# Healthcare-Robotics/assistive-gym

Measured on NVIDIA H100. Metric: env-steps/sec FeedingJaco-v1 @batch4096, higher is better.
Workload: dtype f32

## Files before the change

assistive_gym_b200/csrc/ag_solver.cuh:

```cuda
#pragma once
#include "ag_device.cuh"

#define RS_HDR 16
#define RS_LB 32
#define RS_UNIT 16
#define RS_MAXREC (RS_HDR + 4 * RS_LB)
enum { RM_BOX = 0, RM_CONE = 1, RM_PAD = 2 };

struct alignas(16) v4 { float x, y, z, w; };
AG_HD v4 ldv4(const float* p) { return *(const v4*)p; }
AG_HD void stv4(float* p, v4 a) { *(v4*)p = a; }
AG_HD float i2f_bits(int v) { float f; memcpy(&f, &v, 4); return f; }
AG_HD int f2i_bits(float f) { int v; memcpy(&v, &f, 4); return v; }

AG_HD int rs_null(const SimDev& S) { return S.NDp + 8 * S.nf; }
AG_HD int rs_nv(const SimDev& S) { return (S.NDp + 8 * S.nf + 8 + 31) & ~31; }
AG_HD int rs_dummy(const SimDev& S) { return 3 * S.ND + S.ngr + 3 * S.maxc; }
AG_HD int rs_nlam(const SimDev& S) { return (3 * S.ND + S.ngr + 3 * S.maxc + 1 + 31) & ~31; }
#define RS_CTA_ENVS 8
AG_HD int rs_env_floats(const SimDev& S) { return rs_nv(S) + rs_nlam(S) + 64 + 1024; }
AG_HD int rs_env_stride(const SimDev& S) { return rs_nv(S) + rs_nlam(S) + 8; }
AG_HD int rs_cta_floats(const SimDev& S) { return 1024 + RS_CTA_ENVS * (1024 + rs_env_stride(S)) + 2 * RS_CTA_ENVS; }

AG_HD int link_ref(const SimDev& S, int e, int link) {
// ... 143 lines not shown
  if (kind < 2) {
    if (!AG_LDG(S.link_haslimit + k)) return false;
    if (kind == 0) { float pen = q - AG_LDG(S.link_lower + k); if (pen > 0.f) return false; R.rhs = (-pen * S.erp / dt - qd) * R.dinv; }
    else { float pen = AG_LDG(S.link_upper + k) - q; if (pen > 0.f) return false; R.rhs = (-pen * S.erp / dt + qd) * R.dinv; R.sgn = -1.f; }
  } else {
    int mode = S.motor_mode[k];
    float maxi = S.motor_maxf[k] * dt;
    if (S.motor_fscale) maxi *= ld1(S.motor_fscale, k, N, e);
    if (mode == 0 || !(maxi > 0.f)) return false;
    float vt = (mode == 1) ? (S.motor_kp[k] * (ld1(S.motor_target, k, N, e) - q) / dt + qd - S.motor_kd[k] * qd)
                           : ld1(S.motor_target, k, N, e);
    R.rhs = (vt - qd) * R.dinv; R.lo = -maxi; R.hi = maxi;
  }
  return true;
}
AG_HD bool con_sides(const SimDev& S, int e, int c, int& refA, int& refB, bool& swapped) {
  const int N = S.N;
  int ka = AG_LDG(S.con_link + 2 * c), kb = AG_LDG(S.con_link + 2 * c + 1);
  int ba = AG_LDG(S.link_body + ka), bb = AG_LDG(S.link_body + kb);
  if (S.body_mode[(size_t)ba * N + e] == 0 || S.body_mode[(size_t)bb * N + e] == 0) return false;
  refA = link_ref(S, e, ka); refB = link_ref(S, e, kb);
  swapped = rs_swap_sides(refA, refB);
  if (swapped) { int t = refA; refA = refB; refB = t; }
  return ((refA | refB) & 3) != 0;
}

AG_HD void contact_refs(const SimDev& S, int e, unsigned key, int& refA, int& refB) {
  unsigned pairk = key >> 2;
  int ca = (int)(pairk / (unsigned)S.nc), cb = (int)(pairk % (unsigned)S.nc);
  refA = link_ref(S, e, AG_LDG(S.col_link + ca)); refB = link_ref(S, e, AG_LDG(S.col_link + cb));
  if (rs_swap_sides(refA, refB)) { int t = refA; refA = refB; refB = t | (1 << 30); }
}

AG_HDN inline void rows_body(int e, const SimDev& S, const KP&) {
  const int N = S.N;
  RsCur c; c.pos = 0; c.rs = S.rs_data + (size_t)e * S.rs_cap; c.capf = S.rs_cap; c.over = false;
  int open_key = -1, open_row = -1, open_off = -1;
  for (int pass = 0; pass < 2; pass++) {
    for (int d = 0; d < S.ND; d++) {
      for (int kind = (pass == 0 ? 0 : 2); kind < (pass == 0 ? 2 : 3); kind++) {
        const int r = kind * S.ND + d;
        DofRow R;
        int info = -1;
        if (dof_row(S, e, kind, d, R)) {
          int a = AG_LDG(S.dl_art + d);
          int key = 0x10000 | a;
          if (open_key == key) {
            info = rs_enc(open_off, 1, 1);
            S.row_off[(size_t)open_row * N + e] |= 2; S.row_pair[(size_t)open_row * N + e] = r;
            open_key = -1;
          } else {
            int nd = AG_LDG(S.art_nd + a);
            int o = rs_alloc(S, c, rs_rec_floats(nd > 8 ? 2 : 1));
            if (o >= 0) { info = rs_enc(o, 0, 0); open_key = key; open_row = r; open_off = o; }
          }
        }
        S.row_off[(size_t)r * N + e] = info;
        S.row_pair[(size_t)r * N + e] = -1;
      }
    }
  }
  open_key = -1;
  for (int cc = 0; cc < S.ncon; cc++) {
    int refA, refB; bool sw;
    bool on = con_sides(S, e, cc, refA, refB, sw);
    RsShape h; h.nv = 0;
    if (on) h = rs_shape(S, refA, refB);
    for (int i = 0; i < 6; i += 2) {
      int r = 3 * S.ND + 6 * cc + i;
      int i0 = -1, i1 = -1;
      if (on && h.nv > 0) {
        int o = rs_alloc(S, c, rs_rec_floats(h.nv));
        if (o >= 0) { i0 = rs_enc(o, 0, 1); i1 = rs_enc(o, 1, 1); }
      }
      S.row_off[(size_t)r * N + e] = i0; S.row_off[(size_t)(r + 1) * N + e] = i1;
      S.row_pair[(size_t)r * N + e] = i0 >= 0 ? r + 1 : -1; S.row_pair[(size_t)(r + 1) * N + e] = -1;
    }
  }
  int cnt = S.c_count[e]; if (cnt > S.maxc) cnt = S.maxc;
  int open_slot = -1;
  for (int s = 0; s < cnt; s++) {
    size_t rb = (size_t)s * 4 * N + e;
    int refA = S.s_ref[rb], refB = S.s_ref[rb + N] & ~(1 << 30);
    RsShape h = rs_shape(S, refA, refB);
    int key = rs_shape_key(h);
    int info = -1;
    if (key >= 0) {
      if (open_key == key && open_slot == s - 1) {
        info = rs_enc(open_off, 1, 1);
        S.s_ref[(size_t)(s - 1) * 4 * N + e + 2 * (size_t)N] |= 2;
        open_key = -1;
      } else {
        int o = rs_alloc(S, c, rs_rec_floats(h.nv));
        if (o >= 0) { info = rs_enc(o, 0, 0); open_key = key; open_slot = s; open_off = o; }
      }
    } else open_key = -1;
    S.s_ref[rb + 2 * (size_t)N] = info;
  }
  for (int s = 0; s < cnt; s++) {
    size_t rb = (size_t)s * 4 * N + e;
    int refA = S.s_ref[rb], refB = S.s_ref[rb + N] & ~(1 << 30);
    RsShape h = rs_shape(S, refA, refB);
    int o = -1;
    if (h.nv > 0 && S.s_ref[rb + 2 * (size_t)N] >= 0) o = rs_alloc(S, c, rs_rec_floats(h.nv));
    S.s_ref[rb + 3 * (size_t)N] = o < 0 ? -1 : o / RS_UNIT;
  }
  if (c.pos % 32 != 0) {
    if (c.pos + RS_UNIT <= c.capf) { rs_pad_header(S, c.rs + c.pos, RM_PAD, RS_UNIT); c.pos += RS_UNIT; } else c.over = true;
  }
  S.rs_nfloats[e] = c.over ? (c.pos / 32) * 32 : c.pos;
  if (c.over) S.overflow[e] = 1;
}

AG_HD void rs_finish_box(const SimDev& S, float* rec, int nv, int row, int li, float num, float lo, float hi) {
  float diag = rs_row_diag(rec, nv, row);
  if (diag > 1e-20f) { float dinv = 1.0f / diag; rs_set_row(S, rec, row, li, num * dinv, dinv, lo, hi); }
  else rs_null_row(rec, nv, row);
}

AG_HDN inline void drow_body(int r, int e, const SimDev& S) {
  const int N = S.N;
  const float dt = S.dt;
  int info = S.row_off[(size_t)r * N + e];
  if (info < 0 || (info & 1)) return;
  float* rec = S.rs_data + (size_t)e * S.rs_cap + (size_t)(info >> 2) * RS_UNIT;
  const int r2 = (info & 2) ? S.row_pair[(size_t)r * N + e] : -1;
  if (r < 3 * S.ND) {
    int d = r % S.ND;
    int a = AG_LDG(S.dl_art + d), d0 = AG_LDG(S.art_dl0 + a), nd = AG_LDG(S.art_nd + a), vo = AG_LDG(S.art_voff + a);
    RsShape h; h.nv = nd > 8 ? 2 : 1; h.sl[0] = vo; h.sl[1] = nd > 8 ? vo + 8 : rs_null(S); h.sl[2] = h.sl[3] = rs_null(S);
    rs_header(S, rec, h, RM_BOX);
    rs_zero_blocks(rec, h.nv);
    int dd[2] = {d, 0}; float sg[2] = {1.f, 1.f};
    for (int row = 0; row < (r2 >= 0 ? 2 : 1); row++) {
      int rr = row == 0 ? r : r2;
      int kind = rr / S.ND; dd[row] = rr % S.ND;
      DofRow R;
      if (!dof_row(S, e, kind, dd[row], R)) continue;
      sg[row] = R.sgn;
      for (int i = 0; i < nd; i++) {
        float* q = rs_entry(rec, 0, i, row);
        q[0] = (i == dd[row] - d0) ? R.sgn : 0.f;
        q[1] = R.sgn * S.Minv[((size_t)(d0 + i) * S.ND + dd[row]) * N + e];
      }
// ... 593 lines not shown
```

assistive_gym_b200/csrc/ag_types.h:

```cpp
#pragma once
#include <stdint.h>
#include <stddef.h>

#define AG_MAXND 16
#define AG_MAX_HULL 64
#define AG_CF 20
#define AG_CFR 10

enum {
  CF_PAX = 0, CF_PAY, CF_PAZ, CF_PBX, CF_PBY, CF_PBZ, CF_NX, CF_NY, CF_NZ, CF_DIST,
  CF_RHS_N, CF_DINV_N, CF_RHS_T1, CF_DINV_T1, CF_RHS_T2, CF_DINV_T2, CF_MU, CF_LAM_N, CF_LAM_T1, CF_LAM_T2
};
enum { BK_STATIC = 0, BK_FREE = 1, BK_ART = 2 };

struct SimDev {
  int N;
  float dt; int iters; float erp, contact_erp, slop, resid_thr, contact_thr, lin_damp, ang_damp, vmax;
  int cone, gyro, maxc;
  int nb, nl, nc, npair, ncon, nf, nart, ND, nparts, nmovcol, nmovlink, nalllink, ngr ;
  const int *body_link0, *body_nlinks, *body_kind, *body_idx;
  const float* body_gravity;
  const int *link_body, *link_parent, *link_jtype, *link_dl, *link_haslimit, *link_col0, *link_ncol;
  const float *link_axis, *link_jpos, *link_jquat, *link_com, *link_iquat, *link_inertia, *link_mass, *link_lower, *link_upper;
  const int *col_link, *col_type, *col_v0, *col_nv, *col_p0, *col_np;
// ... 6 lines not shown
  const int* con_link; const float *con_pivot, *con_quat, *con_maxforce;
  const int* free_body; const float* free_invm;
  const int *art_body, *art_dl0, *art_nd, *art_voff;
  int NDp;
  const int *dl_link, *dl_parent, *dl_type, *dl_art, *dl_part0, *dl_nparts;
  const float *dl_mass, *dl_mc, *dl_J, *dl_damping;
  const float *pt_mass, *pt_com, *pt_I;
  int* motor_mode; float *motor_kp, *motor_kd, *motor_maxf;
  int* hard_limit;
  float *motor_target, *motor_applied;
  float* motor_fscale;
  float *base_pos, *base_quat, *base_lin, *base_ang;
  float *jq, *jqd;
  float* friction;
  int* body_mode;
  float *lpos, *lquat;
  float *cmin, *cmax, *lmin, *lmax;
  int* cand_count; unsigned *cand, *cand_s; int maxcand;
  int* c_count;
  int maxraw;
  unsigned *c_key, *s_key;
  float *c_data, *s_data;
  int *s_ref;
  int* overflow;
  float *fcom, *fIinv;
  float *jax, *jor;
  float* Minv;
  float* dv;
  float* dr_lam;
  float* gr_lam;
  int* row_off;
  int* row_pair;
  float* rs_data; int rs_cap; int* rs_nfloats;
  int* iters_used;
  int* pgs_order;
  int* pgs_cycles;
  int* pgs_trips;
};

struct KP {
  int n;
  int i0, i1, i2, i3;
  float f0, f1;
  const void* p0; void* p1; void* p2; void* p3; void* p4; void* p5;
};
```

assistive_gym_b200/csrc/agphys.cu:

```cuda
#include <stdio.h>
#include <stdlib.h>
#include <string.h>
#include <string>
#include <vector>
#include <algorithm>
#include "../../include/agphys.h"
#include "ag_device.cuh"
#include "ag_solver.cuh"
#include "ag_feeding.cuh"
#include "ag_bathing.cuh"
#include "ag_ik.cuh"
#include "ag_cloth.cuh"
#include "ag_dressing.cuh"
#include "ag_render.cuh"
#include "ag_scratch.cuh"
#include "ag_coop.cuh"
#include "ag_drinking.cuh"

#ifndef AG_CPU_EMU
#include <cuda_runtime.h>
#define AG_GLOBAL __global__
#else
#define AG_GLOBAL
typedef void* cudaStream_t;
#endif

static thread_local std::string g_err;
static int fail(const std::string& m) { g_err = m; return -1; }

#ifndef AG_CPU_EMU
#define AG_KERNEL(name, body)                                                   \
  __global__ void __launch_bounds__(128) name(SimDev S, KP p) {                 \
    int tid = blockIdx.x * blockDim.x + threadIdx.x;                            \
    if (tid < p.n) body(tid, S, p);                                             \
  }
#else
#define AG_KERNEL(name, body) \
  static void name(SimDev S, KP p) { for (int tid = 0; tid < p.n; tid++) body(tid, S, p); }
#endif

#ifndef AG_CPU_EMU
#define AG_KERNEL_B(name, body, minblocks)                                      \
  __global__ void __launch_bounds__(128, minblocks) name(SimDev S, KP p) {      \
    int tid = blockIdx.x * blockDim.x + threadIdx.x;                            \
    if (tid < p.n) body(tid, S, p);                                             \
  }
#else
#define AG_KERNEL_B(name, body, minblocks) AG_KERNEL(name, body)
#endif
AG_KERNEL(k_fk, fk_body)
AG_KERNEL(k_aabb, aabb_body)
AG_KERNEL(k_linkaabb, linkaabb_body)
AG_KERNEL(k_pairs, pairs_body)
AG_KERNEL(k_csort, csort_body)
AG_KERNEL_B(k_narrow, narrow_body, 3)
AG_KERNEL(k_sort, sort_body)
AG_KERNEL(k_dyn, dyn_body)
AG_KERNEL(k_rows, rows_body)
AG_KERNEL(k_crows, crows_body)
#ifndef AG_CPU_EMU
__global__ void __launch_bounds__(32) k_pgs(SimDev S, KP p) {
  extern __shared__ __align__(128) float pgs_smem[];
  pgs_warp(S, pgs_smem, p.i0, blockIdx.x * RS_CTA_ENVS);
}
__global__ void __launch_bounds__(1024) k_order(SimDev S, KP) {
  __shared__ int hist[64];
  if (threadIdx.x < 64) hist[threadIdx.x] = 0;
  __syncthreads();
  for (int e = threadIdx.x; e < S.N; e += blockDim.x) atomicAdd(&hist[pgs_work_bucket(S, e)], 1);
  __syncthreads();
  if (threadIdx.x == 0) { int acc = 0; for (int b = 0; b < 64; b++) { int c = hist[b]; hist[b] = acc; acc += c; } }
  __syncthreads();
  for (int e = threadIdx.x; e < S.N; e += blockDim.x) S.pgs_order[atomicAdd(&hist[pgs_work_bucket(S, e)], 1)] = e;
}
#else
static void k_pgs(SimDev S, KP p) {
  std::vector<float> buf((size_t)rs_env_floats(S) + 8);
  float* base = (float*)(((uintptr_t)buf.data() + 15) & ~(uintptr_t)15);
  static const bool emul = getenv("AG_EMU_PLAIN_PGS") == nullptr;
  for (int tid = 0; tid < p.n; tid++) { if (emul) pgs_env_emul(tid, S, base); else pgs_body_host(tid, S, base); }
}
static void k_order(SimDev S, KP) {
  int hist[64] = {0};
  for (int e = 0; e < S.N; e++) hist[pgs_work_bucket(S, e)]++;
  int acc = 0; for (int b = 0; b < 64; b++) { int c = hist[b]; hist[b] = acc; acc += c; }
  for (int e = 0; e < S.N; e++) S.pgs_order[hist[pgs_work_bucket(S, e)]++] = e;
}
#endif
AG_KERNEL(k_integrate, integrate_body)
AG_KERNEL(k_gather, gather_body)
AG_KERNEL(k_scatter, scatter_body)
// ... 49 lines not shown
  const CoopDev& C = *(const CoopDev*)p.p1;
  float h[2 * AG_MLP_H];
  for (int e = 0; e < p.n; e++) coop_limits_body(e, S, C, C.mlp, h, 1);
}
static void k_coop_classify(SimDev, KP p) {
  float h[2 * AG_MLP_H];
  for (int i = 0; i < p.n; i++) {
    const float* xi = (const float*)p.p0 + (size_t)i * 4;
    float x[4] = {xi[0], xi[1], xi[2], xi[3]};
    ((float*)p.p3)[i] = coop_mlp((const float*)p.p2, x, h, 1);
  }
}
#endif

enum Task { TASK_FEEDING = 0, TASK_SCRATCH = 1, TASK_BATHING = 2, TASK_DRESSING = 3, TASK_DRINKING = 4 };
static const int IO_COOP = 5;
static const int ROBOT_OBS_W[5] = {25, 30, 24, 24, 25}, HUMAN_OBS_W[5] = {23, 34, 28, 28, 0};
static const char* const TASK_INIT[5] = {"ag_feeding_init", "ag_scratch_init", "ag_bathing_init", "ag_dressing_init", "ag_drinking_init"};

struct StepOut { float *obs, *obs_h, *reward, *done, *info; };
struct StepGraph { void* exec; const void* key[6]; uint64_t launches; bool valid; };
struct StepIO {
  int act_w, obs_w, obs_h_w;
  float *action, *obs, *obs_h, *reward, *done, *info;
  float *host_in, *host_out;
  StepGraph graph;
};

struct AgSim {
  SimDev S;
  AgConfig cfg;
  int device;
  cudaStream_t stream;
  uint64_t launches;
  std::vector<void*> allocs;
  std::vector<int> body_link0, body_nlinks, body_kind, link_body;
  int nl, nb;
  float* d_stage; size_t stage_floats;
  std::vector<float> h_stage;
  int* d_mask; int* d_links; int* d_icount;
  FeedDev F; FeedDev* F_dev; bool feeding;
  BathDev B; BathDev* B_dev; bool bathing;
  bool bath_frames;
  ClothDev C; ClothDev* C_dev; bool cloth; int cloth_sub, cloth_npt, cloth_qs;
  DressPost DP; DressPost* DP_dev; bool dressing;
  ScratchDev SD; ScratchDev* SD_dev; bool scratch;
  DrinkDev DK; DrinkDev* DK_dev; bool drinking;
  size_t render_pix; int render_n; int* d_render_ids; unsigned char* d_render_rgba; float* d_render_depth; void* d_render_dev;
  CoopDev CO; CoopDev* CO_dev; bool coop;
  StepIO io[6];
  bool use_graph; int graph_failures;
  bool profiling;
  std::vector<std::string> knames;
  std::vector<int> ev_slot;
  std::vector<void*> ev_begin, ev_end;
};

#ifndef AG_CPU_EMU
#define CK(x) do { cudaError_t err__ = (x); if (err__ != cudaSuccess) { g_err = std::string(#x) + ": " + cudaGetErrorString(err__); return -1; } } while (0)
#define CKP(x) do { cudaError_t err__ = (x); if (err__ != cudaSuccess) { g_err = std::string(#x) + ": " + cudaGetErrorString(err__); return nullptr; } } while (0)
#endif

static void drop_graph(StepIO& io) {
#ifndef AG_CPU_EMU
  if (io.graph.valid) { cudaGraphExecDestroy((cudaGraphExec_t)io.graph.exec); io.graph.valid = false; }
#else
// ... 21 lines not shown
#else
  (void)s; memcpy(d, h, bytes);
#endif
  return 0;
}
static int d2h(AgSim* s, void* h, const void* d, size_t bytes) {
#ifndef AG_CPU_EMU
  CK(cudaMemcpyAsync(h, d, bytes, cudaMemcpyDeviceToHost, s->stream));
  CK(cudaStreamSynchronize(s->stream));
#else
  (void)s; memcpy(h, d, bytes);
#endif
  return 0;
}
static int dev_zero(AgSim* s, void* d, size_t bytes) {
#ifndef AG_CPU_EMU
  CK(cudaMemsetAsync(d, 0, bytes, s->stream));
#else
  (void)s; memset(d, 0, bytes);
#endif
  return 0;
}
template <typename T>
static const T* upload(AgSim* s, const std::vector<T>& v) {
  T* d = (T*)dev_alloc(s, v.size() * sizeof(T));
  if (d && !v.empty()) h2d(s, d, v.data(), v.size() * sizeof(T));
  return d;
}
template <typename T>
static T* dalloc(AgSim* s, size_t n) { return (T*)dev_alloc(s, n * sizeof(T)); }

#define AG_MAX_KNAMES 32
static int prof_slot(AgSim* s, const char* name);
static void prof_mark(AgSim* s, int slot, bool begin);
#ifndef AG_CPU_EMU
#define LAUNCH(sim, kern, nthreads, kp)                                                     \
  do {                                                                                      \
    KP kp__ = (kp); kp__.n = (int)(nthreads);                                               \
    if (kp__.n > 0) {                                                                       \
      int ps__ = (sim)->profiling ? prof_slot((sim), #kern) : -1;                           \
      if (ps__ >= 0) prof_mark((sim), ps__, true);                                          \
      kern<<<(kp__.n + 127) / 128, 128, 0, (sim)->stream>>>((sim)->S, kp__);                \
      if (ps__ >= 0) prof_mark((sim), ps__, false);                                         \
      (sim)->launches++;                                                                    \
    }                                                                                       \
  } while (0)
#else
#define LAUNCH(sim, kern, nthreads, kp) \
  do { KP kp__ = (kp); kp__.n = (int)(nthreads); if (kp__.n > 0) { kern((sim)->S, kp__); (sim)->launches++; } } while (0)
#endif

static int prof_slot(AgSim* s, const char* name) {
  for (size_t i = 0; i < s->knames.size(); i++) if (s->knames[i] == name) return (int)i;
  if (s->knames.size() >= AG_MAX_KNAMES) return -1;
  s->knames.push_back(name);
  return (int)s->knames.size() - 1;
}
static void prof_mark(AgSim* s, int slot, bool begin) {
#ifndef AG_CPU_EMU
  cudaEvent_t ev;
  if (cudaEventCreate(&ev) != cudaSuccess) return;
  cudaEventRecord(ev, s->stream);
  if (begin) { s->ev_slot.push_back(slot); s->ev_begin.push_back((void*)ev); } else s->ev_end.push_back((void*)ev);
#else
  (void)s; (void)slot; (void)begin;
#endif
}

static KP kp0() { KP p; memset(&p, 0, sizeof(p)); return p; }

struct DevGuard {
  int prev;
  explicit DevGuard(int device) : prev(-1) {
#ifndef AG_CPU_EMU
    if (cudaGetDevice(&prev) != cudaSuccess) prev = -1;
    if (prev != device) cudaSetDevice(device); else prev = -1;
#else
    (void)device;
#endif
  }
  ~DevGuard() {
#ifndef AG_CPU_EMU
    if (prev >= 0) cudaSetDevice(prev);
#endif
  }
};

struct HQ { double x, y, z, w; };
static HQ hq_mul(HQ a, HQ b) {
  return HQ{a.w * b.x + a.x * b.w + a.y * b.z - a.z * b.y, a.w * b.y - a.x * b.z + a.y * b.w + a.z * b.x,
            a.w * b.z + a.x * b.y - a.y * b.x + a.z * b.w, a.w * b.w - a.x * b.x - a.y * b.y - a.z * b.z};
}
static void hq_mat(HQ q, double R[9]) {
  double x = q.x, y = q.y, z = q.z, w = q.w;
  R[0] = 1 - 2 * (y * y + z * z); R[1] = 2 * (x * y - z * w); R[2] = 2 * (x * z + y * w);
  R[3] = 2 * (x * y + z * w); R[4] = 1 - 2 * (x * x + z * z); R[5] = 2 * (y * z - x * w);
  R[6] = 2 * (x * z - y * w); R[7] = 2 * (y * z + x * w); R[8] = 1 - 2 * (x * x + y * y);
}

extern "C" {

const char* ag_last_error(void) { return g_err.c_str(); }

void ag_default_config(AgConfig* c) {
  c->dt = 0.02; c->num_substeps = 1; c->num_solver_iters = 50; c->erp = 0.2; c->contact_erp = 0.08;
  c->linear_slop = 1e-5; c->residual_threshold = 1e-7; c->contact_threshold = 0.02;
  c->linear_damping = 0.04; c->angular_damping = 0.04; c->max_coord_velocity = 100; c->hull_margin = 0.001;
  c->cone_friction = 1; c->gyroscopic = 1; c->max_contacts = 128;
  c->warmstart_contact = 0.0; c->warmstart_joint = 0.0;
}

AgSim* ag_create(const AgSceneDesc* d, const AgConfig* cfg, int n_envs, int device) {
  if (!d || !cfg || n_envs <= 0) { g_err = "ag_create: bad arguments"; return nullptr; }
  DevGuard guard__(device);
  AgSim* s = new AgSim();
  memset(&s->S, 0, sizeof(SimDev));
  memset(&s->F, 0, sizeof(FeedDev));
  s->cfg = *cfg; s->device = device; s->launches = 0; s->feeding = false; s->bathing = false; s->cloth = false; s->cloth_sub = 0; s->C_dev = nullptr; s->dressing = false; s->DP_dev = nullptr; s->scratch = false; s->SD_dev = nullptr; s->drinking = false; s->DK_dev = nullptr; s->render_pix = 0; s->render_n = 0; s->d_render_ids = nullptr; s->d_render_rgba = nullptr; s->d_render_depth = nullptr; s->d_render_dev = nullptr; s->use_graph = true; s->graph_failures = 0; s->coop = false; s->CO_dev = nullptr; s->B_dev = nullptr; s->stream = nullptr; s->F_dev = nullptr; s->profiling = false;
  s->d_stage = nullptr; s->stage_floats = 0;
#ifndef AG_CPU_EMU
  { int ndev = 0; if (cudaGetDeviceCount(&ndev) != cudaSuccess || device < 0 || device >= ndev) { g_err = "no such CUDA device (is a CUDA device present? there is no CPU fallback)"; delete s; return nullptr; } }
  if (cudaStreamCreateWithFlags(&s->stream, cudaStreamNonBlocking) != cudaSuccess) { g_err = "cudaStreamCreate failed"; delete s; return nullptr; }
#endif
  SimDev& S = s->S;
  const int N = n_envs;
  S.N = N;
  int sub = cfg->num_substeps > 0 ? cfg->num_substeps : 1;
  S.dt = (float)(cfg->dt / sub); S.iters = cfg->num_solver_iters; S.erp = (float)cfg->erp; S.contact_erp = (float)cfg->contact_erp;
  S.slop = (float)cfg->linear_slop; S.resid_thr = (float)cfg->residual_threshold; S.contact_thr = (float)cfg->contact_threshold;
  S.lin_damp = (float)cfg->linear_damping; S.ang_damp = (float)cfg->angular_damping; S.vmax = (float)cfg->max_coord_velocity;
  S.cone = cfg->cone_friction; S.gyro = cfg->gyroscopic; S.maxc = cfg->max_contacts > 0 ? cfg->max_contacts : 128;
  const int nb = d->n_bodies, nl = d->n_links, nc = d->n_colliders;
  S.nb = nb; S.nl = nl; S.nc = nc; S.npair = d->n_pairs; S.ncon = d->n_constraints;
  s->nb = nb; s->nl = nl;
  s->body_link0.assign(d->body_link0, d->body_link0 + nb);
  s->body_nlinks.assign(d->body_nlinks, d->body_nlinks + nb);
  s->link_body.assign(d->link_body, d->link_body + nl);

  std::vector<double> subtree(nl, 0.0);
  for (int k = nl - 1; k >= 0; k--) { subtree[k] += d->link_mass[k]; if (d->link_parent[k] >= 0) subtree[d->link_parent[k]] += subtree[k]; }
  std::vector<int> live(nl, 0), link_dl(nl, -1), body_kind(nb, BK_STATIC), body_idx(nb, -1);
  std::vector<int> free_body, art_body, art_dl0, art_nd, dl_link, dl_parent, dl_type, dl_art, dl_part0, dl_nparts;
  std::vector<float> dl_mass, dl_mc, dl_J, dl_damping, pt_mass, pt_com, pt_I;
  for (int b = 0; b < nb; b++) {
    int l0 = d->body_link0[b], nlk = d->body_nlinks[b];
    int nlive = 0;
    for (int k = l0 + 1; k < l0 + nlk; k++) {
      int jt = d->link_jtype[k];
      if ((jt == AG_JOINT_REVOLUTE || jt == AG_JOINT_PRISMATIC) && subtree[k] > 0) { live[k] = 1; nlive++; }
    }
    if (d->link_jtype[l0] == AG_JOINT_FREE_BASE && d->link_mass[l0] > 0) {
      if (nlive > 0) { g_err = "floating-base articulated bodies are not supported yet"; ag_destroy(s); return nullptr; }
      body_kind[b] = BK_FREE; body_idx[b] = (int)free_body.size(); free_body.push_back(b);
    } else if (nlive > 0) {
      body_kind[b] = BK_ART; body_idx[b] = (int)art_body.size();
// ... 128 lines not shown
  S.dl_link = upload(s, dl_link); S.dl_parent = upload(s, dl_parent); S.dl_type = upload(s, dl_type); S.dl_art = upload(s, dl_art);
  S.dl_part0 = upload(s, dl_part0); S.dl_nparts = upload(s, dl_nparts);
  S.dl_mass = upload(s, dl_mass); S.dl_mc = upload(s, dl_mc); S.dl_J = upload(s, dl_J); S.dl_damping = upload(s, dl_damping);
  S.pt_mass = upload(s, pt_mass); S.pt_com = upload(s, pt_com); S.pt_I = upload(s, pt_I);
  S.hard_limit = dalloc<int>(s, nl);
  S.motor_mode = dalloc<int>(s, nl); S.motor_kp = dalloc<float>(s, nl); S.motor_kd = dalloc<float>(s, nl); S.motor_maxf = dalloc<float>(s, nl);
  S.motor_target = dalloc<float>(s, (size_t)nl * N); S.motor_applied = dalloc<float>(s, (size_t)nl * N);
  S.base_pos = dalloc<float>(s, (size_t)nb * 3 * N); S.base_quat = dalloc<float>(s, (size_t)nb * 4 * N);
  S.base_lin = dalloc<float>(s, (size_t)nb * 3 * N); S.base_ang = dalloc<float>(s, (size_t)nb * 3 * N);
  S.jq = dalloc<float>(s, (size_t)nl * N); S.jqd = dalloc<float>(s, (size_t)nl * N);
  S.friction = dalloc<float>(s, (size_t)nl * N); S.body_mode = dalloc<int>(s, (size_t)nb * N);
  S.lpos = dalloc<float>(s, (size_t)nl * 3 * N); S.lquat = dalloc<float>(s, (size_t)nl * 4 * N);
  S.cmin = dalloc<float>(s, (size_t)nc * 3 * N); S.cmax = dalloc<float>(s, (size_t)nc * 3 * N);
  S.lmin = dalloc<float>(s, (size_t)nl * 3 * N); S.lmax = dalloc<float>(s, (size_t)nl * 3 * N);
  S.c_count = dalloc<int>(s, N); S.overflow = dalloc<int>(s, N); S.iters_used = dalloc<int>(s, N); S.pgs_cycles = dalloc<int>(s, N); S.pgs_trips = dalloc<int>(s, N);
  S.pgs_order = dalloc<int>(s, N);
  S.maxcand = 4 * S.maxc; S.cand_count = dalloc<int>(s, N); S.cand = dalloc<unsigned>(s, (size_t)S.maxcand * N); S.cand_s = dalloc<unsigned>(s, (size_t)S.maxcand * N);
  if ((size_t)nc * nc >= (1u << 24)) { g_err = "too many colliders (pair id must fit 24 bits)"; ag_destroy(s); return nullptr; }
  S.maxraw = 4 * S.maxc;
  S.c_key = dalloc<unsigned>(s, (size_t)S.maxraw * N); S.s_key = dalloc<unsigned>(s, (size_t)S.maxc * N);
  S.c_data = dalloc<float>(s, (size_t)S.maxraw * AG_CFR * N); S.s_data = dalloc<float>(s, (size_t)S.maxc * AG_CF * N);
  S.s_ref = dalloc<int>(s, (size_t)S.maxc * 4 * N);
  S.fcom = dalloc<float>(s, (size_t)S.nf * 3 * N); S.fIinv = dalloc<float>(s, (size_t)S.nf * 6 * N);
  S.jax = dalloc<float>(s, (size_t)S.ND * 3 * N); S.jor = dalloc<float>(s, (size_t)S.ND * 3 * N);
  S.Minv = dalloc<float>(s, (size_t)S.ND * S.ND * N);
  S.dv = dalloc<float>(s, (size_t)(S.ND + 6 * S.nf) * N);
  S.dr_lam = dalloc<float>(s, (size_t)3 * S.ND * N);
  {
    size_t fl = (size_t)(3 * S.ND / 2 + 2) * rs_rec_floats(2) + (size_t)3 * S.ncon * rs_rec_floats(3) + (size_t)S.maxc * 2 * rs_rec_floats(2);
    fl = fl + fl * 3 / 10 + 1024;
    S.rs_cap = (int)((fl + 1023) / 1024 * 1024);
  }
  if (rs_nv(S) + 8 >= 65536 || rs_nlam(S) >= 65536) { g_err = "solver index space exceeds 16 bits: lower max_contacts"; ag_destroy(s); return nullptr; }
  S.rs_data = dalloc<float>(s, (size_t)S.rs_cap * N); S.rs_nfloats = dalloc<int>(s, N);
  S.gr_lam = dalloc<float>(s, (size_t)S.ngr * N); S.row_off = dalloc<int>(s, (size_t)(3 * S.ND + S.ngr) * N); S.row_pair = dalloc<int>(s, (size_t)(3 * S.ND + S.ngr) * N);
  s->d_mask = dalloc<int>(s, N); s->d_links = dalloc<int>(s, 1024); s->d_icount = dalloc<int>(s, N);
  if (!S.gr_lam || !S.rs_data || !S.rs_nfloats || !S.row_pair || !S.s_data) { g_err = "device allocation failed"; ag_destroy(s); return nullptr; }
#ifndef AG_CPU_EMU
  {
    { const char* gg = getenv("AG_GRAPH"); if (gg && atoi(gg) == 0) s->use_graph = false; }
    size_t smem = (size_t)rs_cta_floats(S) * sizeof(float);
    if (smem > 227 * 1024) { g_err = "PGS shared-memory footprint exceeds 227 KB per CTA: lower max_contacts"; ag_destroy(s); return nullptr; }
    if (cudaFuncSetAttribute(k_pgs, cudaFuncAttributeMaxDynamicSharedMemorySize, (int)smem) != cudaSuccess) { g_err = "cudaFuncSetAttribute(k_pgs) failed"; ag_destroy(s); return nullptr; }
  }
#endif
  {
    std::vector<float> fr((size_t)nl * N);
    for (int k = 0; k < nl; k++) for (int e = 0; e < N; e++) fr[(size_t)k * N + e] = (float)d->link_friction[k];
    h2d(s, S.friction, fr.data(), fr.size() * sizeof(float));
    std::vector<int> md((size_t)nb * N, 1);
    h2d(s, S.body_mode, md.data(), md.size() * sizeof(int));
    std::vector<float> q((size_t)nb * 4 * N, 0.f);
    for (int b = 0; b < nb; b++) for (int e = 0; e < N; e++) q[((size_t)b * 4 + 3) * N + e] = 1.f;
    h2d(s, S.base_quat, q.data(), q.size() * sizeof(float));
  }
  return s;
}

void ag_destroy(AgSim* s) {
  if (!s) return;
  DevGuard guard__(s->device);
#ifndef AG_CPU_EMU
  if (s->stream) cudaStreamSynchronize(s->stream);
  for (void* p : s->allocs) cudaFree(p);
  for (StepIO& io : s->io) {
    cudaFreeHost(io.host_in); cudaFreeHost(io.host_out);
    if (io.graph.valid) cudaGraphExecDestroy((cudaGraphExec_t)io.graph.exec);
  }
  if (s->stream) cudaStreamDestroy(s->stream);
#else
  for (void* p : s->allocs) free(p);
  for (StepIO& io : s->io) { free(io.host_in); free(io.host_out); }
#endif
  delete s;
}

int ag_num_envs(const AgSim* s) {
  DevGuard guard__(s->device); return s->S.N; }
void* ag_stream(AgSim* s) {
  DevGuard guard__(s->device); return (void*)s->stream; }
uint64_t ag_kernel_launches(const AgSim* s) {
  DevGuard guard__(s->device); return s->launches; }

int ag_profile_enable(AgSim* s, int on) {
  DevGuard guard__(s->device);
  s->profiling = on != 0;
  return 0;
}
int ag_profile_get(AgSim* s, int max_names, char* names, int name_stride, float* total_ms, int32_t* counts) {
  DevGuard guard__(s->device);
  int n = (int)s->knames.size();
  if (n > max_names) n = max_names;
  for (int i = 0; i < n; i++) { total_ms[i] = 0.f; counts[i] = 0; snprintf(names + (size_t)i * name_stride, name_stride, "%s", s->knames[i].c_str()); }
#ifndef AG_CPU_EMU
  CK(cudaStreamSynchronize(s->stream));
  size_t m = std::min(s->ev_begin.size(), s->ev_end.size());
  for (size_t i = 0; i < m; i++) {
    float ms = 0.f;
    cudaEventElapsedTime(&ms, (cudaEvent_t)s->ev_begin[i], (cudaEvent_t)s->ev_end[i]);
    int sl = s->ev_slot[i];
    if (sl < n) { total_ms[sl] += ms; counts[sl] += 1; }
// ... 123 lines not shown
  if (h2d(s, s->S.motor_mode, mm.data(), sizeof(int) * s->nl) || h2d(s, s->S.motor_kp, a.data(), sizeof(float) * s->nl) ||
      h2d(s, s->S.motor_kd, b.data(), sizeof(float) * s->nl) || h2d(s, s->S.motor_maxf, c.data(), sizeof(float) * s->nl)) return -1;
  if (target) return scatter_host(s, s->S.motor_target, 1, n, links, target, nullptr);
  return 0;
}
int ag_set_motor_force_scale(AgSim* s, int n, const int32_t* links, const float* scale) {
  DevGuard guard__(s->device);
  if (!s->S.motor_fscale) {
    const size_t cnt = (size_t)s->nl * s->S.N;
    s->S.motor_fscale = dalloc<float>(s, cnt);
    if (!s->S.motor_fscale) return fail("device allocation failed");
    std::vector<float> ones(cnt, 1.0f);
    if (h2d(s, s->S.motor_fscale, ones.data(), cnt * sizeof(float))) return -1;
    drop_all_graphs(s);
  }
  return scatter_host(s, s->S.motor_fscale, 1, n, links, scale, nullptr);
}
int ag_set_motor_targets_dev(AgSim* s, int n, const int32_t* links, const float* target_dev) {
  DevGuard guard__(s->device);
  if (n > 1024) return fail("too many items");
  if (check_items(s, s->S.motor_target, n, links)) return -1;
  if (h2d(s, s->d_links, links, sizeof(int) * n)) return -1;
  KP p = kp0(); p.i0 = 1; p.i1 = n; p.p0 = target_dev; p.p1 = s->S.motor_target; p.p2 = s->d_links; p.p3 = nullptr;
  LAUNCH(s, k_scatter, (size_t)s->S.N * n, p);
  return 0;
}

int ag_set_motor_targets_host(AgSim* s, int n, const int32_t* links, const float* target) {
  DevGuard guard__(s->device);
  return scatter_host(s, s->S.motor_target, 1, n, links, target, nullptr);
}

static void cloth_launch(AgSim* s);
static void substep(AgSim* s) {
  SimDev& S = s->S;
  const int N = S.N;
  KP z = kp0();
  LAUNCH(s, k_fk, (size_t)S.nb * N, z);
  if (s->cloth) {
    KP cs = kp0(); cs.p0 = s->C_dev; cs.i0 = s->cloth_sub;
    LAUNCH(s, k_cloth_snap, (size_t)s->C.ncl * N, cs);
  }
  KP a = kp0(); a.p0 = S.movcol; a.i0 = S.nmovcol;
  LAUNCH(s, k_aabb, (size_t)S.nmovcol * N, a);
  KP l = kp0(); l.p0 = S.movlink; l.i0 = S.nmovlink;
  LAUNCH(s, k_linkaabb, (size_t)S.nmovlink * N, l);
  dev_zero(s, S.c_count, sizeof(int) * N);
  dev_zero(s, S.cand_count, sizeof(int) * N);
  int Npad = (N + 31) / 32 * 32;
  KP c = kp0(); c.i0 = Npad;
  LAUNCH(s, k_pairs, (size_t)S.nslice * Npad, c);
  LAUNCH(s, k_csort, (size_t)S.maxcand * N, z);
  LAUNCH(s, k_narrow, (size_t)S.maxcand * N, z);
  LAUNCH(s, k_sort, (size_t)S.maxraw * N, z);
  LAUNCH(s, k_dyn, (size_t)(S.nf + S.nart) * N, z);
  LAUNCH(s, k_rows, N, z);
  LAUNCH(s, k_crows, (size_t)(S.maxc + 3 * S.ND + S.ngr) * N, z);
#ifndef AG_CPU_EMU
  {
    int ps = s->profiling ? prof_slot(s, "k_order") : -1;
    if (ps >= 0) prof_mark(s, ps, true);
    k_order<<<1, 1024, 0, s->stream>>>(S, z);
    if (ps >= 0) prof_mark(s, ps, false);
    KP kp = z; kp.n = N;
    size_t smem = (size_t)rs_cta_floats(S) * sizeof(float);
    ps = s->profiling ? prof_slot(s, "k_pgs") : -1;
    if (ps >= 0) prof_mark(s, ps, true);
    k_pgs<<<(N + RS_CTA_ENVS - 1) / RS_CTA_ENVS, 32, smem, s->stream>>>(S, kp);
    if (ps >= 0) prof_mark(s, ps, false);
    s->launches += 2;
  }
#else
  k_order(S, z);
  LAUNCH(s, k_pgs, N, z);
  LAUNCH(s, k_integrate, N, z);
#endif
  if (s->cloth && ++s->cloth_sub == s->C.K) { s->cloth_sub = 0; cloth_launch(s); }
}

int ag_step(AgSim* s, int n_steps) {
  DevGuard guard__(s->device);
  int sub = s->cfg.num_substeps > 0 ? s->cfg.num_substeps : 1;
  for (int i = 0; i < n_steps * sub; i++) substep(s);
  KP z = kp0();
  LAUNCH(s, k_fk, (size_t)s->S.nb * s->S.N, z);
#ifndef AG_CPU_EMU
  CK(cudaGetLastError());
#endif
  return 0;
}

int ag_get_joint_states(AgSim* s, int n, const int32_t* links, float* q, float* qd, float* tau) {
  DevGuard guard__(s->device);
  if (q && gather_host(s, s->S.jq, 1, n, links, q)) return -1;
  if (qd && gather_host(s, s->S.jqd, 1, n, links, qd)) return -1;
  if (tau && gather_host(s, s->S.motor_applied, 1, n, links, tau)) return -1;
  return 0;
}

int ag_get_link_states(AgSim* s, int n, const int32_t* links, float* pos, float* quat, float* com_pos, float* com_quat, float* lin_vel, float* ang_vel) {
  DevGuard guard__(s->device);
  const int N = s->S.N;
// ... 206 lines not shown
static int* task_male(const AgSim* s, Task task) {
  switch (task) {
    case TASK_FEEDING: return s->F.male;
    case TASK_SCRATCH: return s->SD.male;
    case TASK_BATHING: return s->B.male;
    case TASK_DRESSING: return s->DP.D.male;
    case TASK_DRINKING: return s->DK.male;
  }
  return nullptr;
}

static int io_alloc(AgSim* s, StepIO& io, int act_w, int obs_w, int obs_h_w) {
  const size_t N = s->S.N;
  io.act_w = act_w; io.obs_w = obs_w; io.obs_h_w = obs_h_w;
  io.action = dalloc<float>(s, N * act_w); io.obs = dalloc<float>(s, N * obs_w);
  io.obs_h = obs_h_w ? dalloc<float>(s, N * obs_h_w) : nullptr;
  io.reward = dalloc<float>(s, N); io.done = dalloc<float>(s, N); io.info = dalloc<float>(s, N * 4);
  if (!io.action || !io.obs || (obs_h_w && !io.obs_h) || !io.reward || !io.done || !io.info) return fail("device allocation failed");
  const size_t in = sizeof(float) * N * act_w, out = sizeof(float) * N * (obs_w + obs_h_w + 6);
#ifndef AG_CPU_EMU
  CK(cudaMallocHost((void**)&io.host_in, in));
  CK(cudaMallocHost((void**)&io.host_out, out));
#else
  io.host_in = (float*)malloc(in); io.host_out = (float*)malloc(out);
#endif
  return 0;
}

static size_t coop_smem_bytes(bool mlp) { return mlp ? (size_t)(AG_MLP_FLOATS + 2 * AG_MLP_H * AG_COOP_T) * sizeof(float) : 0; }
static void coop_limits_launch(AgSim* s) {
  KP p = kp0(); p.n = s->S.N; p.p1 = s->CO_dev;
#ifndef AG_CPU_EMU
  int ps = s->profiling ? prof_slot(s, "k_coop_limits") : -1;
  if (ps >= 0) prof_mark(s, ps, true);
  k_coop_limits<<<(p.n + AG_COOP_T - 1) / AG_COOP_T, AG_COOP_T, coop_smem_bytes(s->CO.mlp_on), s->stream>>>(s->S, p);
  if (ps >= 0) prof_mark(s, ps, false);
#else
  k_coop_limits(s->S, p);
#endif
  s->launches++;
}

static int fused_enqueue(AgSim* s, Task task, bool coop, const float* action, const StepOut& o) {
  const int N = s->S.N, k = coop ? s->CO.P.n_ctrl : 0;
  void* dev = task_dev(s, task);
  KP p = kp0(); p.p0 = action; p.p1 = dev; p.i0 = k;
  switch (task) {
    case TASK_FEEDING: LAUNCH(s, k_feed_pre, N, p); break;
    case TASK_SCRATCH: LAUNCH(s, k_scratch_pre, N, p); break;
    case TASK_BATHING: LAUNCH(s, k_bath_pre, N, p); break;
    case TASK_DRESSING: LAUNCH(s, k_dress_pre, N, p); break;
    case TASK_DRINKING: LAUNCH(s, k_drink_pre, N, p); break;
  }
  if (coop) {
    KP c = kp0(); c.p0 = action; c.p1 = s->CO_dev;
    LAUNCH(s, k_coop_pre, N, c);
  }
  const int sub = s->cfg.num_substeps > 0 ? s->cfg.num_substeps : 1;
  const int frames = coop ? s->CO.frame_skip : task_frame_skip(s, task);
  KP z = kp0();
  for (int f = 0; f < frames; f++) {
    for (int i = 0; i < sub; i++) substep(s);
    if (coop) coop_limits_launch(s);
    if (task == TASK_DRESSING) {
      LAUNCH(s, k_fk, (size_t)s->S.nb * N, z);
      KP a = kp0(); a.p0 = s->C_dev; a.i0 = s->DP.D.P.ee_link;
      LAUNCH(s, k_cloth_follow, N, a);
    }
  }
// ... 98 lines not shown
  const float* src[5] = {io.obs, io.obs_h, io.reward, io.done, io.info};
  const int w[5] = {io.obs_w, io.obs_h_w, 1, 1, 4};
  float* h = io.host_out;
  for (int i = 0; i < 5; h += N * w[i], i++) if (w[i] && copy_async(s, h, src[i], sizeof(float) * N * w[i])) return -1;
  return 0;
}
static int host_end(AgSim* s, Task task, bool coop, const StepOut& o) {
  if (step_check(s, task, coop)) return -1;
  const StepIO& io = step_io(s, task, coop);
#ifndef AG_CPU_EMU
  CK(cudaStreamSynchronize(s->stream));
  CK(cudaGetLastError());
#endif
  const size_t N = s->S.N;
  float* dst[5] = {o.obs, o.obs_h, o.reward, o.done, o.info};
  const int w[5] = {io.obs_w, io.obs_h_w, 1, 1, 4};
  const float* h = io.host_out;
  for (int i = 0; i < 5; h += N * w[i], i++) if (w[i] && dst[i]) memcpy(dst[i], h, sizeof(float) * N * w[i]);
  return 0;
}
static int host_step(AgSim* s, Task task, bool coop, const float* action, const StepOut& o) {
  return host_begin(s, task, coop, action) ? -1 : host_end(s, task, coop, o);
}

static size_t cloth_smem_bytes(const AgSim* s) {
  size_t f = (size_t)4 * s->cloth_npt * AG_CLOTH_T + AG_CLOTH_LKS * AG_CLOTH_MAXCL + 12 * (size_t)s->C.maxcc + 40 + 192;
  if (s->cloth_qs) f += (size_t)4 * s->cloth_npt * AG_CLOTH_T;
  return f * sizeof(float);
}
static void cloth_launch(AgSim* s) {
#ifndef AG_CPU_EMU
  size_t smem = cloth_smem_bytes(s);
  int ps = s->profiling ? prof_slot(s, "k_cloth") : -1;
  if (ps >= 0) prof_mark(s, ps, true);
  if (s->cloth_npt == 4) { if (s->cloth_qs) k_cloth<4, true><<<s->S.N, AG_CLOTH_T, smem, s->stream>>>(s->S, s->C); else k_cloth<4, false><<<s->S.N, AG_CLOTH_T, smem, s->stream>>>(s->S, s->C); }
  else { if (s->cloth_qs) k_cloth<8, true><<<s->S.N, AG_CLOTH_T, smem, s->stream>>>(s->S, s->C); else k_cloth<8, false><<<s->S.N, AG_CLOTH_T, smem, s->stream>>>(s->S, s->C); }
  if (ps >= 0) prof_mark(s, ps, false);
#else
  for (int e = 0; e < s->S.N; e++) cloth_env_host(s->S, s->C, e);
#endif
  s->launches++;
}

int ag_cloth_init(AgSim* s, const AgClothDesc* d) {
  DevGuard guard__(s->device);
  if (s->cloth) return fail("ag_cloth_init: the sim already has a cloth");
  if (!d || d->n_nodes <= 0 || d->n_nodes > 65535) return fail("ag_cloth_init: 1..65535 nodes");
  if (d->n_nodes > 8 * AG_CLOTH_T) return fail("ag_cloth_init: more than 8192 nodes");
  if (d->n_colours < 1 || d->n_colours > AG_CLOTH_MAXCOL) return fail("ag_cloth_init: 1..16 link colours");
  if (d->n_anchors < 0 || d->n_anchors > AG_CLOTH_MAXANCH) return fail("ag_cloth_init: at most 8 anchors");
  if (d->n_col_links < 0 || d->n_col_links > AG_CLOTH_MAXCL) return fail("ag_cloth_init: at most 96 collider links");
  const int N = s->S.N, nn = d->n_nodes;
  ClothDev& C = s->C;
  memset(&C, 0, sizeof(C));
  C.nn = nn; C.nlinks = d->n_links; C.ncol = d->n_colours; C.nanch = d->n_anchors; C.ncl = d->n_col_links;
  s->cloth_npt = nn <= 4 * AG_CLOTH_T ? 4 : 8;
  C.nnp = (nn + 31) / 32 * 32;
  C.maxcc = d->max_contacts > 0 ? d->max_contacts : 1024;
  C.K = s->cfg.num_substeps > 0 ? s->cfg.num_substeps : 1;
  C.piters = d->piterations; C.export_contacts = 1;
  C.dt = s->S.dt; C.im = (float)d->inv_mass; C.kLSTh = (float)(0.5 * d->kLST); C.kDP = (float)d->kDP; C.kDG = (float)d->kDG; C.kLF = (float)d->kLF;
  C.kDF = (float)d->kDF; C.kCHR = (float)d->kCHR; C.kKHR = (float)d->kKHR; C.kAHR = (float)d->kAHR; C.margin = (float)d->margin; C.density = (float)d->air_density;
  C.gx = (float)d->gravity[0]; C.gy = (float)d->gravity[1]; C.gz = (float)d->gravity[2];
  for (int c = 0; c <= d->n_colours; c++) C.col_off[c] = d->colour_off[c];
  if (C.col_off[0] != 0 || C.col_off[d->n_colours] != d->n_links) return fail("ag_cloth_init: colour offsets do not cover the link list");
  std::vector<unsigned> lij(d->n_links); std::vector<float> lr(d->n_links);
  {
    std::vector<int> seen(nn, -1);
    for (int c = 0; c < d->n_colours; c++)
      for (int l = C.col_off[c]; l < C.col_off[c + 1]; l++) {
// ... 571 lines not shown
```

Measured before the change: 365,600.

## Fork joint dynamics and row setup onto side stream, overlapping collision pipeline

Splits the per-env row-setup kernel into a joint/constraint part and a contact part. The joint part is fused into the dynamics kernel: the last-arriving thread per env, found with an atomic counter, builds the joint rows. Dynamics plus joint rows run on a second stream forked after FK, concurrently with the collision kernels, and the main stream joins before contact rows. The aim is to fill GPU idle time from small serial launches, at the cost of atomics, extra fences, and cross-stream event dependencies inside the captured graph.

Result: faster. 380,000 (median of 6 runs) (+3.9%).

```diff
diff --git a/assistive_gym_b200/csrc/ag_solver.cuh b/assistive_gym_b200/csrc/ag_solver.cuh
--- a/assistive_gym_b200/csrc/ag_solver.cuh
+++ b/assistive_gym_b200/csrc/ag_solver.cuh
@@ -199,7 +199,8 @@
   if (rs_swap_sides(refA, refB)) { int t = refA; refA = refB; refB = t | (1 << 30); }
 }
 
-AG_HDN inline void rows_body(int e, const SimDev& S, const KP&) {
+#define RS_JCUR_OVER (1 << 30)
+AG_HDN inline void rows_joint_body(int e, const SimDev& S, const KP&) {
   const int N = S.N;
   RsCur c; c.pos = 0; c.rs = S.rs_data + (size_t)e * S.rs_cap; c.capf = S.rs_cap; c.over = false;
   int open_key = -1, open_row = -1, open_off = -1;
@@ -244,6 +245,13 @@
       S.row_pair[(size_t)r * N + e] = i0 >= 0 ? r + 1 : -1; S.row_pair[(size_t)(r + 1) * N + e] = -1;
     }
   }
+  S.rs_jcur[e] = c.pos | (c.over ? RS_JCUR_OVER : 0);
+}
+AG_HDN inline void rows_contact_body(int e, const SimDev& S, const KP&) {
+  const int N = S.N;
+  const int jc = S.rs_jcur[e];
+  RsCur c; c.pos = jc & ~RS_JCUR_OVER; c.rs = S.rs_data + (size_t)e * S.rs_cap; c.capf = S.rs_cap; c.over = (jc & RS_JCUR_OVER) != 0;
+  int open_key = -1, open_off = -1;
   int cnt = S.c_count[e]; if (cnt > S.maxc) cnt = S.maxc;
   int open_slot = -1;
   for (int s = 0; s < cnt; s++) {
@@ -277,6 +285,25 @@
   }
   S.rs_nfloats[e] = c.over ? (c.pos / 32) * 32 : c.pos;
   if (c.over) S.overflow[e] = 1;
+}
+
+AG_HD bool ag_last_arrival(int* cnt, int n) {
+#if defined(__CUDA_ARCH__)
+  __threadfence();
+  if (atomicAdd(cnt, 1) != n - 1) return false;
+  *cnt = 0;
+  __threadfence();
+  return true;
+#else
+  if (++*cnt != n) return false;
+  *cnt = 0;
+  return true;
+#endif
+}
+AG_HDN inline void dyn_rows_body(int tid, const SimDev& S, const KP& p) {
+  dyn_body(tid, S, p);
+  const int e = tid % S.N;
+  if (ag_last_arrival(S.dyn_arrive + e, S.nf + S.nart)) rows_joint_body(e, S, p);
 }
 
 AG_HD void rs_finish_box(const SimDev& S, float* rec, int nv, int row, int li, float num, float lo, float hi) {
diff --git a/assistive_gym_b200/csrc/ag_types.h b/assistive_gym_b200/csrc/ag_types.h
--- a/assistive_gym_b200/csrc/ag_types.h
+++ b/assistive_gym_b200/csrc/ag_types.h
@@ -62,6 +62,8 @@
   int* row_off;
   int* row_pair;
   float* rs_data; int rs_cap; int* rs_nfloats;
+  int* rs_jcur;
+  int* dyn_arrive;
   int* iters_used;
   int* pgs_order;
   int* pgs_cycles;
diff --git a/assistive_gym_b200/csrc/agphys.cu b/assistive_gym_b200/csrc/agphys.cu
--- a/assistive_gym_b200/csrc/agphys.cu
+++ b/assistive_gym_b200/csrc/agphys.cu
@@ -55,8 +55,9 @@
 AG_KERNEL(k_csort, csort_body)
 AG_KERNEL_B(k_narrow, narrow_body, 3)
 AG_KERNEL(k_sort, sort_body)
-AG_KERNEL(k_dyn, dyn_body)
-AG_KERNEL(k_rows, rows_body)
+AG_KERNEL(k_dyn, dyn_rows_body)
+AG_KERNEL(k_rows_joint, rows_joint_body)
+AG_KERNEL(k_rows_contact, rows_contact_body)
 AG_KERNEL(k_crows, crows_body)
 #ifndef AG_CPU_EMU
 __global__ void __launch_bounds__(32) k_pgs(SimDev S, KP p) {
@@ -172,6 +173,8 @@
   AgConfig cfg;
   int device;
   cudaStream_t stream;
+  cudaStream_t side; void *fork_ev, *join_ev; bool fork;
+  bool emu_collide_first;
   uint64_t launches;
   std::vector<void*> allocs;
   std::vector<int> body_link0, body_nlinks, body_kind, link_body;
@@ -259,23 +262,24 @@
 
 #define AG_MAX_KNAMES 32
 static int prof_slot(AgSim* s, const char* name);
-static void prof_mark(AgSim* s, int slot, bool begin);
-#ifndef AG_CPU_EMU
-#define LAUNCH(sim, kern, nthreads, kp)                                                     \
+static void prof_mark(AgSim* s, cudaStream_t st, int slot, bool begin);
+#ifndef AG_CPU_EMU
+#define LAUNCH_ON(sim, st, kern, nthreads, kp)                                              \
   do {                                                                                      \
     KP kp__ = (kp); kp__.n = (int)(nthreads);                                               \
     if (kp__.n > 0) {                                                                       \
       int ps__ = (sim)->profiling ? prof_slot((sim), #kern) : -1;                           \
-      if (ps__ >= 0) prof_mark((sim), ps__, true);                                          \
-      kern<<<(kp__.n + 127) / 128, 128, 0, (sim)->stream>>>((sim)->S, kp__);                \
-      if (ps__ >= 0) prof_mark((sim), ps__, false);                                         \
+      if (ps__ >= 0) prof_mark((sim), (st), ps__, true);                                    \
+      kern<<<(kp__.n + 127) / 128, 128, 0, (st)>>>((sim)->S, kp__);                         \
+      if (ps__ >= 0) prof_mark((sim), (st), ps__, false);                                   \
       (sim)->launches++;                                                                    \
     }                                                                                       \
   } while (0)
 #else
-#define LAUNCH(sim, kern, nthreads, kp) \
-  do { KP kp__ = (kp); kp__.n = (int)(nthreads); if (kp__.n > 0) { kern((sim)->S, kp__); (sim)->launches++; } } while (0)
-#endif
+#define LAUNCH_ON(sim, st, kern, nthreads, kp) \
+  do { (void)(st); KP kp__ = (kp); kp__.n = (int)(nthreads); if (kp__.n > 0) { kern((sim)->S, kp__); (sim)->launches++; } } while (0)
+#endif
+#define LAUNCH(sim, kern, nthreads, kp) LAUNCH_ON(sim, (sim)->stream, kern, nthreads, kp)
 
 static int prof_slot(AgSim* s, const char* name) {
   for (size_t i = 0; i < s->knames.size(); i++) if (s->knames[i] == name) return (int)i;
@@ -283,14 +287,14 @@
   s->knames.push_back(name);
   return (int)s->knames.size() - 1;
 }
-static void prof_mark(AgSim* s, int slot, bool begin) {
+static void prof_mark(AgSim* s, cudaStream_t st, int slot, bool begin) {
 #ifndef AG_CPU_EMU
   cudaEvent_t ev;
   if (cudaEventCreate(&ev) != cudaSuccess) return;
-  cudaEventRecord(ev, s->stream);
+  cudaEventRecord(ev, st);
   if (begin) { s->ev_slot.push_back(slot); s->ev_begin.push_back((void*)ev); } else s->ev_end.push_back((void*)ev);
 #else
-  (void)s; (void)slot; (void)begin;
+  (void)s; (void)st; (void)slot; (void)begin;
 #endif
 }
 
@@ -344,10 +348,20 @@
   memset(&s->S, 0, sizeof(SimDev));
   memset(&s->F, 0, sizeof(FeedDev));
   s->cfg = *cfg; s->device = device; s->launches = 0; s->feeding = false; s->bathing = false; s->cloth = false; s->cloth_sub = 0; s->C_dev = nullptr; s->dressing = false; s->DP_dev = nullptr; s->scratch = false; s->SD_dev = nullptr; s->drinking = false; s->DK_dev = nullptr; s->render_pix = 0; s->render_n = 0; s->d_render_ids = nullptr; s->d_render_rgba = nullptr; s->d_render_depth = nullptr; s->d_render_dev = nullptr; s->use_graph = true; s->graph_failures = 0; s->coop = false; s->CO_dev = nullptr; s->B_dev = nullptr; s->stream = nullptr; s->F_dev = nullptr; s->profiling = false;
+  s->side = nullptr; s->fork_ev = nullptr; s->join_ev = nullptr; s->fork = true;
+  { const char* sf = getenv("AG_SUBSTEP_FORK"); if (sf && atoi(sf) == 0) s->fork = false; }
+  { const char* cf = getenv("AG_EMU_COLLIDE_FIRST"); s->emu_collide_first = cf && atoi(cf) != 0; }
   s->d_stage = nullptr; s->stage_floats = 0;
 #ifndef AG_CPU_EMU
   { int ndev = 0; if (cudaGetDeviceCount(&ndev) != cudaSuccess || device < 0 || device >= ndev) { g_err = "no such CUDA device (is a CUDA device present? there is no CPU fallback)"; delete s; return nullptr; } }
   if (cudaStreamCreateWithFlags(&s->stream, cudaStreamNonBlocking) != cudaSuccess) { g_err = "cudaStreamCreate failed"; delete s; return nullptr; }
+  {
+    cudaEvent_t f = nullptr, j = nullptr;
+    const bool ok = cudaStreamCreateWithFlags(&s->side, cudaStreamNonBlocking) == cudaSuccess && cudaEventCreateWithFlags(&f, cudaEventDisableTiming) == cudaSuccess &&
+                    cudaEventCreateWithFlags(&j, cudaEventDisableTiming) == cudaSuccess;
+    s->fork_ev = (void*)f; s->join_ev = (void*)j;
+    if (!ok) { g_err = "cudaStreamCreate / cudaEventCreate failed"; ag_destroy(s); return nullptr; }
+  }
 #endif
   SimDev& S = s->S;
   const int N = n_envs;
@@ -542,10 +556,10 @@
     S.rs_cap = (int)((fl + 1023) / 1024 * 1024);
   }
   if (rs_nv(S) + 8 >= 65536 || rs_nlam(S) >= 65536) { g_err = "solver index space exceeds 16 bits: lower max_contacts"; ag_destroy(s); return nullptr; }
-  S.rs_data = dalloc<float>(s, (size_t)S.rs_cap * N); S.rs_nfloats = dalloc<int>(s, N);
+  S.rs_data = dalloc<float>(s, (size_t)S.rs_cap * N); S.rs_nfloats = dalloc<int>(s, N); S.rs_jcur = dalloc<int>(s, N); S.dyn_arrive = dalloc<int>(s, N);
   S.gr_lam = dalloc<float>(s, (size_t)S.ngr * N); S.row_off = dalloc<int>(s, (size_t)(3 * S.ND + S.ngr) * N); S.row_pair = dalloc<int>(s, (size_t)(3 * S.ND + S.ngr) * N);
   s->d_mask = dalloc<int>(s, N); s->d_links = dalloc<int>(s, 1024); s->d_icount = dalloc<int>(s, N);
-  if (!S.gr_lam || !S.rs_data || !S.rs_nfloats || !S.row_pair || !S.s_data) { g_err = "device allocation failed"; ag_destroy(s); return nullptr; }
+  if (!S.gr_lam || !S.rs_data || !S.rs_nfloats || !S.rs_jcur || !S.dyn_arrive || !S.row_pair || !S.s_data) { g_err = "device allocation failed"; ag_destroy(s); return nullptr; }
 #ifndef AG_CPU_EMU
   {
     { const char* gg = getenv("AG_GRAPH"); if (gg && atoi(gg) == 0) s->use_graph = false; }
@@ -577,6 +591,9 @@
     cudaFreeHost(io.host_in); cudaFreeHost(io.host_out);
     if (io.graph.valid) cudaGraphExecDestroy((cudaGraphExec_t)io.graph.exec);
   }
+  if (s->side) { cudaStreamSynchronize(s->side); cudaStreamDestroy(s->side); }
+  if (s->fork_ev) cudaEventDestroy((cudaEvent_t)s->fork_ev);
+  if (s->join_ev) cudaEventDestroy((cudaEvent_t)s->join_ev);
   if (s->stream) cudaStreamDestroy(s->stream);
 #else
   for (void* p : s->allocs) free(p);
@@ -766,15 +783,13 @@
 }
 
 static void cloth_launch(AgSim* s);
-static void substep(AgSim* s) {
+#ifdef AG_CPU_EMU
+static void (*g_emu_substep_hook)(AgSim*, int stage) = nullptr;
+#endif
+static void substep_collide(AgSim* s) {
   SimDev& S = s->S;
   const int N = S.N;
   KP z = kp0();
-  LAUNCH(s, k_fk, (size_t)S.nb * N, z);
-  if (s->cloth) {
-    KP cs = kp0(); cs.p0 = s->C_dev; cs.i0 = s->cloth_sub;
-    LAUNCH(s, k_cloth_snap, (size_t)s->C.ncl * N, cs);
-  }
   KP a = kp0(); a.p0 = S.movcol; a.i0 = S.nmovcol;
   LAUNCH(s, k_aabb, (size_t)S.nmovcol * N, a);
   KP l = kp0(); l.p0 = S.movlink; l.i0 = S.nmovlink;
@@ -787,21 +802,57 @@
   LAUNCH(s, k_csort, (size_t)S.maxcand * N, z);
   LAUNCH(s, k_narrow, (size_t)S.maxcand * N, z);
   LAUNCH(s, k_sort, (size_t)S.maxraw * N, z);
-  LAUNCH(s, k_dyn, (size_t)(S.nf + S.nart) * N, z);
-  LAUNCH(s, k_rows, N, z);
+}
+static void substep_joint(AgSim* s, cudaStream_t st) {
+  SimDev& S = s->S;
+  const int N = S.N;
+  KP z = kp0();
+  if (S.nf + S.nart > 0) LAUNCH_ON(s, st, k_dyn, (size_t)(S.nf + S.nart) * N, z);
+  else LAUNCH_ON(s, st, k_rows_joint, N, z);
+}
+static void substep(AgSim* s) {
+  SimDev& S = s->S;
+  const int N = S.N;
+  KP z = kp0();
+  LAUNCH(s, k_fk, (size_t)S.nb * N, z);
+  if (s->cloth) {
+    KP cs = kp0(); cs.p0 = s->C_dev; cs.i0 = s->cloth_sub;
+    LAUNCH(s, k_cloth_snap, (size_t)s->C.ncl * N, cs);
+  }
+#ifndef AG_CPU_EMU
+  if (s->fork && !s->profiling) {
+    cudaEventRecord((cudaEvent_t)s->fork_ev, s->stream);
+    cudaStreamWaitEvent(s->side, (cudaEvent_t)s->fork_ev, 0);
+    substep_joint(s, s->side);
+    cudaEventRecord((cudaEvent_t)s->join_ev, s->side);
+    substep_collide(s);
+    cudaStreamWaitEvent(s->stream, (cudaEvent_t)s->join_ev, 0);
+  } else {
+    substep_joint(s, s->stream);
+    substep_collide(s);
+  }
+#else
+  if (s->emu_collide_first) { substep_collide(s); substep_joint(s, s->stream); }
+  else { substep_joint(s, s->stream); substep_collide(s); }
+  if (g_emu_substep_hook) g_emu_substep_hook(s, 0);
+#endif
+  LAUNCH(s, k_rows_contact, N, z);
   LAUNCH(s, k_crows, (size_t)(S.maxc + 3 * S.ND + S.ngr) * N, z);
+#ifdef AG_CPU_EMU
+  if (g_emu_substep_hook) g_emu_substep_hook(s, 1);
+#endif
 #ifndef AG_CPU_EMU
   {
     int ps = s->profiling ? prof_slot(s, "k_order") : -1;
-    if (ps >= 0) prof_mark(s, ps, true);
+    if (ps >= 0) prof_mark(s, s->stream, ps, true);
     k_order<<<1, 1024, 0, s->stream>>>(S, z);
-    if (ps >= 0) prof_mark(s, ps, false);
+    if (ps >= 0) prof_mark(s, s->stream, ps, false);
     KP kp = z; kp.n = N;
     size_t smem = (size_t)rs_cta_floats(S) * sizeof(float);
     ps = s->profiling ? prof_slot(s, "k_pgs") : -1;
-    if (ps >= 0) prof_mark(s, ps, true);
+    if (ps >= 0) prof_mark(s, s->stream, ps, true);
     k_pgs<<<(N + RS_CTA_ENVS - 1) / RS_CTA_ENVS, 32, smem, s->stream>>>(S, kp);
-    if (ps >= 0) prof_mark(s, ps, false);
+    if (ps >= 0) prof_mark(s, s->stream, ps, false);
     s->launches += 2;
   }
 #else
@@ -1074,9 +1125,9 @@
   KP p = kp0(); p.n = s->S.N; p.p1 = s->CO_dev;
 #ifndef AG_CPU_EMU
   int ps = s->profiling ? prof_slot(s, "k_coop_limits") : -1;
-  if (ps >= 0) prof_mark(s, ps, true);
+  if (ps >= 0) prof_mark(s, s->stream, ps, true);
   k_coop_limits<<<(p.n + AG_COOP_T - 1) / AG_COOP_T, AG_COOP_T, coop_smem_bytes(s->CO.mlp_on), s->stream>>>(s->S, p);
-  if (ps >= 0) prof_mark(s, ps, false);
+  if (ps >= 0) prof_mark(s, s->stream, ps, false);
 #else
   k_coop_limits(s->S, p);
 #endif
@@ -1241,10 +1292,10 @@
 #ifndef AG_CPU_EMU
   size_t smem = cloth_smem_bytes(s);
   int ps = s->profiling ? prof_slot(s, "k_cloth") : -1;
-  if (ps >= 0) prof_mark(s, ps, true);
+  if (ps >= 0) prof_mark(s, s->stream, ps, true);
   if (s->cloth_npt == 4) { if (s->cloth_qs) k_cloth<4, true><<<s->S.N, AG_CLOTH_T, smem, s->stream>>>(s->S, s->C); else k_cloth<4, false><<<s->S.N, AG_CLOTH_T, smem, s->stream>>>(s->S, s->C); }
   else { if (s->cloth_qs) k_cloth<8, true><<<s->S.N, AG_CLOTH_T, smem, s->stream>>>(s->S, s->C); else k_cloth<8, false><<<s->S.N, AG_CLOTH_T, smem, s->stream>>>(s->S, s->C); }
-  if (ps >= 0) prof_mark(s, ps, false);
+  if (ps >= 0) prof_mark(s, s->stream, ps, false);
 #else
   for (int e = 0; e < s->S.N; e++) cloth_env_host(s->S, s->C, e);
 #endif
```
